# jaak-s/BayesianDataFusion.jl

Measured on AMD Instinct MI355X. Metric: Gibbs sweeps/sec (both entities) + test RMSE, MovieLens-1M D=32, higher is better.
Workload: dtype f64; 1 GPU; BPMF MovieLens-1M 6040x3952, 500209 training ratings (500000 held out), D=32, alpha=1.5, step = rows of both entities + hyperpriors + test prediction update (one native call); BEFORE the --warmup steps the engine's set-up runs 60 ms of full iterations whose results are discarded (device_warmup_ms); num_latent=32, burnin=5, psamples=1985, parallelism=1 GPU

## Files before the change

### bayesiandatafusion.jl_amd/csrc/dpp_rows32.h

```cpp
#pragma once
#include "dpp_rows16.h"

namespace {

template <int S, int I>
__device__ __forceinline__ int sys_off(int j)
{
    constexpr int IB = I / 16, ii = I % 16;
    if constexpr (IB >= S) {
        constexpr int blk = IB * (IB + 1) / 2 + S;
        return (blk * 4 + (ii >> 2)) * 64 + 16 * (ii & 3) + j;
    } else {
        return (1 * 4 + (j >> 2)) * 64 + 16 * (j & 3) + ii;
    }
}

template <int DR, int I>
__device__ __forceinline__ void col_rank1(double (&A0)[33], double (&A1)[33], double v0, double v1)
{
    if constexpr (I < 16) {
        if constexpr (I == 0) fm1<0>(A0[0], v0, v0); else fm1_run<I>(A0[I], v0, v0);
        if constexpr (16 + I < DR) {
            fm1_run<I>(A0[16 + I], v1, v0);
            fm1_run<I>(A1[16 + I], v1, v1);
        }
        col_rank1<DR, I + 1>(A0, A1, v0, v1);
    }
}
template <int DR, int S, int K, int I, bool FIRST>
__device__ __forceinline__ void fin_elim(double (&A0)[33], double (&A1)[33], double nm0, double nm1)
{
    if constexpr (I <= 32) {
        if constexpr (S == 0) {
            if constexpr (DR > 16) {
                if constexpr (FIRST) fm1<K>(A1[I], A0[I], nm1); else fm1_run<K>(A1[I], A0[I], nm1);
                fm1_self_run<K>(A0[I], nm0);
            } else {
                if constexpr (FIRST) fm1_self<K>(A0[I], nm0); else fm1_self_run<K>(A0[I], nm0);
            }
        } else {
            if constexpr (FIRST) fm1_self<K>(A1[I], nm1); else fm1_self_run<K>(A1[I], nm1);
        }
        fin_elim<DR, S, K, (I + 1 < DR || I == 32) ? I + 1 : 32, false>(A0, A1, nm0, nm1);
    }
}

template <int DR, int k>
__device__ __forceinline__ void fin_factor(double (&A0)[33], double (&A1)[33], double &d0, double &d1, int j)
{
    if constexpr (k < DR) {
        constexpr int S = k / 16, K = k % 16;
        const double dk = row_bcast_f64<K>(S ? A1[k] : A0[k]);
        const double rinv = fast_rcp(dk);
        double nm0 = 0.0, nm1;
        if constexpr (S == 0) {
            d0 = (j == K) ? dk : d0;
            nm0 = (j > K) ? -(A0[k] * rinv) : 0.0;
            nm1 = -(A1[k] * rinv);
        } else {
            d1 = (j == K) ? dk : d1;
            nm1 = (j > K) ? -(A1[k] * rinv) : 0.0;
        }
        fin_elim<DR, S, K, (k + 1 < DR) ? k + 1 : 32, true>(A0, A1, nm0, nm1);
        fin_factor<DR, k + 1>(A0, A1, d0, d1, j);
    }
}

template <int C>
__device__ __forceinline__ void fin_backward(const double (&A0)[33], const double (&A1)[33], double &y0, double &y1, double rd0,
                                             double rd1, int j)
{
    if constexpr (C >= 1) {
        constexpr int S = C / 16, K = C % 16;
        if constexpr (S == 1) {
            fm1<K>(y0, y1, -(A0[C] * rd0));
            if constexpr (K > 0) fm1_self_run<K>(y1, (j < K) ? -(A1[C] * rd1) : 0.0);
        } else {
            fm1_self<K>(y0, (j < K) ? -(A0[C] * rd0) : 0.0);
        }
        fin_backward<C - 1>(A0, A1, y0, y1, rd0, rd1, j);
    }
}

}
```

### bayesiandatafusion.jl_amd/csrc/k_rows_col.hip

```cpp
#include "rows.h"
#include "dpp_rows32.h"
#include <algorithm>

#ifndef BDF_COL_WAVES
#define BDF_COL_WAVES 2
#endif
#define COL_VGPR_HALF 104
#define COL_PSZ 800

#ifdef BDF_K1_STAMPS
#define CSTAMP_DECL unsigned long long st_t = __builtin_amdgcn_s_memtime(), st_acc = 0, st_mid = 0, st_prior = 0, st_fin = 0, st_rng = 0, st_steps = 0, st_rounds = 0, st_parts = 0, st_fins = 0, st_folds = 0; const unsigned long long st_begin = st_t
#define CSTAMP(x) do { const unsigned long long now_ = __builtin_amdgcn_s_memtime(); x += now_ - st_t; st_t = now_; } while (0)
#else
#define CSTAMP_DECL do { } while (0)
#define CSTAMP(x) do { } while (0)
#endif

namespace {

struct ColCoef { static __device__ __forceinline__ double c(double x) { asm volatile("" : "+s"(x)); return x; } };

template <int DR, int K>
__device__ __forceinline__ void col_obs(double (&A0)[33], double (&A1)[33], double v0, double v1, double r)
{
    col_rank1<DR, 0>(A0, A1, v0, v1);
    fm1_run<K>(A0[32], r, v0);
    fm1_run<K>(A1[32], r, v1);
}

__device__ __forceinline__ double col_ld(__amdgpu_buffer_rsrc_t rs, uint32_t off)
{
    typedef unsigned u2v __attribute__((ext_vector_type(2)));
    const u2v x = __builtin_amdgcn_raw_buffer_load_b64(rs, (int)off, 0, 0);
    return __hiloint2double((int)x.y, (int)x.x);
}

template <bool FULL, int K0>
__device__ __forceinline__ void col_gather4(double (&b)[4][2], __amdgpu_buffer_rsrc_t rs, uint32_t idw, uint32_t rowb, uint32_t eo, bool ok1)
{
#pragma unroll
    for (int q = 0; q < 4; q++) {
        uint32_t id;
        if (q == 0) id = row_bcast_u32<K0>(idw); else if (q == 1) id = row_bcast_u32<K0 + 1>(idw);
        else if (q == 2) id = row_bcast_u32<K0 + 2>(idw); else id = row_bcast_u32<K0 + 3>(idw);
        if constexpr (FULL) {
            const uint32_t base = id + eo;
            b[q][1] = col_ld(rs, base);
            b[q][0] = col_ld(rs, base + 128u);
        } else {
            const uint32_t base = id + eo;
            b[q][0] = col_ld(rs, base);
            b[q][1] = col_ld(rs, ok1 ? base - 128u : 0xffffffffu);
        }
    }
}
template <int DR, int K0>
__device__ __forceinline__ void col_compute4(double (&A0)[33], double (&A1)[33], const double (&b)[4][2], double r)
{
    col_obs<DR, K0>(A0, A1, b[0][0], b[0][1], r);
    col_obs<DR, K0 + 1>(A0, A1, b[1][0], b[1][1], r);
    col_obs<DR, K0 + 2>(A0, A1, b[2][0], b[2][1], r);
    col_obs<DR, K0 + 3>(A0, A1, b[3][0], b[3][1], r);
}

template <int X>
__device__ __forceinline__ void col_fold(double (&A0)[33], double (&A1)[33], double m)
{
#pragma unroll
    for (int i = 0; i < 33; i++) A0[i] = fma(__shfl_xor(A0[i], X), m, A0[i]);
#pragma unroll
    for (int i = 16; i < 33; i++) A1[i] = fma(__shfl_xor(A1[i], X), m, A1[i]);
}

template <int E0, int E1, bool ADD>
__device__ __forceinline__ void col_slot_load(double (&A0)[33], double (&A1)[33], const double *src, double m)
{
#pragma unroll
    for (int e = E0; e < E1; e++) {
        const double v = src[e * 16];
        double &d = e < 33 ? A0[e] : A1[e - 17];
        if (ADD) d = fma(v, m, d); else d = v * m;
    }
}

__device__ __forceinline__ void col_prior_dma(const double *image, unsigned lds_dst, int lane)
{
    const void *sbase = (const void *)(((uint64_t)(uint32_t)__builtin_amdgcn_readfirstlane((int)((uint64_t)image >> 32)) << 32) |
                                       (uint32_t)__builtin_amdgcn_readfirstlane((int)(uint32_t)(uint64_t)image));
#pragma unroll
    for (int k = 0; k < 6; k++) {
        const unsigned voff = (unsigned)k * 1024u + (unsigned)lane * 16u;
        unsigned keep;
        asm volatile("s_mov_b32 %0, m0\n\ts_mov_b32 m0, %2\n\ts_nop 0\n\tglobal_load_lds_dwordx4 %1, %3 sc1\n\ts_mov_b32 m0, %0"
                     : "=&s"(keep) : "v"(voff), "s"(lds_dst + (unsigned)k * 1024u), "s"(sbase) : "memory");
    }
}
template <int S, int I, int DR>
__device__ __forceinline__ void col_prior_lds(double (&A)[33], const double *img, double alpha, int j)
{
    if constexpr (I < DR) {
        A[I] = fma(alpha, A[I], img[sys_off<S, I>(j)]);
        col_prior_lds<S, I + 1, DR>(A, img, alpha, j);
    }
}

template <int DR, bool FULL>
__global__ __launch_bounds__(64, BDF_COL_WAVES) __attribute__((amdgpu_num_vgpr(COL_VGPR_HALF))) void k_rows_col(SampleArgs a_in, ColPlanDev p_in, uint32_t fac_bytes)
{
    __shared__ __attribute__((aligned(16))) double lds[4 * 272 + 768];
    const int w = blockIdx.x;
    if (w >= p_in.n_waves) return;
    const int r_end = p_in.wave_round[w + 1];
    if (a_in.span && threadIdx.x == 0) atomicMin(a_in.span + 2 * (w & 63), (unsigned long long)__builtin_amdgcn_s_memrealtime());
    CSTAMP_DECL;
#pragma nounroll
    for (int rd = p_in.wave_round[w]; rd < r_end; rd++) {
    int zero = 0, lane = threadIdx.x;
    asm volatile("" : "+s"(zero), "+v"(lane));
    const SampleArgs &a = (&a_in)[zero];
    const ColPlanDev &p = (&p_in)[zero];
    const int j = lane & 15, g = lane >> 4;
    const TermDev &T = a.t[0];
    const int D = FULL ? 32 : a.D;
    const int ec0 = D - 1 - j, ec1 = D - 17 - j;
    const int n0 = ec0, n1 = ec1 >= 0 ? ec1 : 0;
    const bool ok1 = ec1 >= 0;
    const uint32_t rowb = (uint32_t)D * 8u;
    const uint32_t eo = FULL ? (uint32_t)ec1 * 8u : (uint32_t)ec0 * 8u;
    const __amdgpu_buffer_rsrc_t rs = __builtin_amdgcn_make_buffer_rsrc((void *)T.fac[0], 0, (int)fac_bytes, 0x00020000);
    const bool coded = T.packed != nullptr;
    const double mean = T.mean;
    {
        const ColJob jb = p.jobs[(int64_t)rd * 4 + g];
        const bool live = jb.row >= 0;
        const int n = live ? jb.count : 0;
        const unsigned lds_img = (unsigned)__builtin_amdgcn_readfirstlane((int)(unsigned)(size_t)(__attribute__((address_space(3))) double *)(lds + 4 * 272));
        bool have_prior = true;
        if (a.ready) have_prior = __builtin_amdgcn_readfirstlane((int)((int32_t)(__hip_atomic_load(a.ready, __ATOMIC_RELAXED, __HIP_MEMORY_SCOPE_AGENT) - a.ready_want) >= 0)) != 0;
        if (have_prior) col_prior_dma(a.prior_c, lds_img, lane);
        double A0[33], A1[33];
#pragma unroll
        for (int i = 0; i < 33; i++) { A0[i] = 0.0; A1[i] = 0.0; }
        int nmax = n;
        nmax = max(nmax, __shfl_xor(nmax, 16));
        nmax = max(nmax, __shfl_xor(nmax, 32));
        nmax = __builtin_amdgcn_readfirstlane(nmax);
        if (nmax > 0) {
            const uint32_t *packed = coded ? T.packed + jb.q_begin : nullptr;
            const int32_t *colidx = T.colidx + jb.q_begin;
            const double *vals = T.vals + jb.q_begin;
            const double *table = T.table;
#define COL_CHUNK(c0, IDW, R)                                                                     \
            {                                                                                     \
                const int o_ = (c0) + j;                                                          \
                IDW = 0xffffffu; R = 0.0;                                                         \
                if (o_ < n) {                                                                     \
                    if (coded) { const uint32_t pw_ = packed[o_]; IDW = pw_; R = table[pw_ >> 24] - mean; } \
                    else { IDW = (uint32_t)colidx[o_]; R = vals[o_] - mean; }                     \
                }                                                                                 \
                IDW = __umul24(IDW, rowb);       \
            }
            uint32_t idw_c, idw_n;
            double r_c, r_n;
            COL_CHUNK(0, idw_c, r_c)
            double ba[4][2], bb[4][2];
            col_gather4<FULL, 0>(ba, rs, idw_c, rowb, eo, ok1);
            for (int c0 = 0;; c0 += 16) {
                COL_CHUNK(c0 + 16, idw_n, r_n)
                col_gather4<FULL, 4>(bb, rs, idw_c, rowb, eo, ok1);
                __builtin_amdgcn_sched_barrier(0);
                col_compute4<DR, 0>(A0, A1, ba, r_c);
                if (c0 + 4 >= nmax) break;
                col_gather4<FULL, 8>(ba, rs, idw_c, rowb, eo, ok1);
                __builtin_amdgcn_sched_barrier(0);
                col_compute4<DR, 4>(A0, A1, bb, r_c);
                if (c0 + 8 >= nmax) break;
                col_gather4<FULL, 12>(bb, rs, idw_c, rowb, eo, ok1);
                __builtin_amdgcn_sched_barrier(0);
                col_compute4<DR, 8>(A0, A1, ba, r_c);
                if (c0 + 12 >= nmax) break;
                col_gather4<FULL, 0>(ba, rs, idw_n, rowb, eo, ok1);
                __builtin_amdgcn_sched_barrier(0);
                col_compute4<DR, 12>(A0, A1, bb, r_c);
                if (c0 + 16 >= nmax) break;
                idw_c = idw_n; r_c = r_n;
            }
#undef COL_CHUNK
        }
#ifdef BDF_K1_STAMPS
        asm volatile("s_nop 0" :: "v"(A0[0]), "v"(A0[32]), "v"(A1[31]));
        st_steps += (unsigned long long)nmax; st_rounds++;
#endif
        CSTAMP(st_acc);
        const unsigned fl = (unsigned)jb.flags;
        if (__builtin_amdgcn_readfirstlane((int)(__ballot((fl & COLF_PAIR) != 0) != 0ull))) {
#ifdef BDF_K1_STAMPS
            st_folds++;
#endif
            col_fold<16>(A0, A1, (fl & COLF_PAIR) ? 1.0 : 0.0);
            if (__builtin_amdgcn_readfirstlane((int)(__ballot((fl & COLF_QUAD) != 0) != 0ull)))
                col_fold<32>(A0, A1, (fl & COLF_QUAD) ? 1.0 : 0.0);
        }
        if (__builtin_amdgcn_readfirstlane((int)(fl & COLF_MULTI))) {
            const int srow = __builtin_amdgcn_readfirstlane(jb.srow);
            double *dst = p.partials + (int64_t)__builtin_amdgcn_readfirstlane(jb.slot) * COL_PSZ + j;
            if (g == 0) {
#pragma unroll
                for (int e = 0; e < 33; e++) __hip_atomic_store(dst + e * 16, A0[e], __ATOMIC_RELAXED, __HIP_MEMORY_SCOPE_AGENT);
#pragma unroll
                for (int e = 33; e < 50; e++) __hip_atomic_store(dst + e * 16, A1[e - 17], __ATOMIC_RELAXED, __HIP_MEMORY_SCOPE_AGENT);
            }
            const ColSplit sr = p.rows[srow];
            asm volatile("s_waitcnt vmcnt(0)" ::: "memory");
            int old = 0;
            if (lane == 0) old = __hip_atomic_fetch_add(p.arrived + srow, 1, __ATOMIC_RELAXED, __HIP_MEMORY_SCOPE_AGENT);
            old = __builtin_amdgcn_readfirstlane(old);
#ifdef BDF_K1_STAMPS
            st_parts++;
            if (old == sr.n_slots - 1) st_fins++;
#endif
            if (old != sr.n_slots - 1) { CSTAMP(st_mid); continue; }
            __builtin_amdgcn_fence(__ATOMIC_ACQUIRE, "agent");
            asm volatile("s_waitcnt vmcnt(0)" ::: "memory");
            if (lane == 0) p.arrived[srow] = 0;
            const double *src = p.partials + (int64_t)sr.slot_begin * COL_PSZ + j;
            col_slot_load<0, 50, false>(A0, A1, src + (int64_t)(g < sr.n_slots ? g : 0) * COL_PSZ, g < sr.n_slots ? 1.0 : 0.0);
            for (int s0 = 4; s0 < sr.n_slots; s0 += 4) {
                const bool on = s0 + g < sr.n_slots;
                const double *sp = src + (int64_t)(on ? s0 + g : 0) * COL_PSZ;
                const double m = on ? 1.0 : 0.0;
                col_slot_load<0, 16, true>(A0, A1, sp, m);
                asm volatile("" ::: "memory");
                col_slot_load<16, 33, true>(A0, A1, sp, m);
                asm volatile("" ::: "memory");
                col_slot_load<33, 50, true>(A0, A1, sp, m);
                asm volatile("" ::: "memory");
            }
            col_fold<16>(A0, A1, 1.0);
            col_fold<32>(A0, A1, 1.0);
        }
        CSTAMP(st_mid);
        double z0 = 0.0, z1 = 0.0;
        {
            double ze = 0.0, zo = 0.0;
            if (live && 2 * j < D) bdf_normal_pair<ColCoef>(a.seed, a.sweep, BDF_P_ROW, a.entity_tag, (uint64_t)(uint32_t)jb.orig, (uint32_t)j, ze, zo);
            const int base = lane & 48;
            const double ze0 = __shfl(ze, base + (n0 >> 1)), zo0 = __shfl(zo, base + (n0 >> 1));
            const double ze1 = __shfl(ze, base + (n1 >> 1)), zo1 = __shfl(zo, base + (n1 >> 1));
            z0 = (n0 & 1) ? zo0 : ze0;
            z1 = ok1 ? ((n1 & 1) ? zo1 : ze1) : 0.0;
        }
        asm volatile("" ::: "memory");
        CSTAMP(st_rng);
        {
            double *tl = lds + g * 272;
#pragma unroll
            for (int r = 0; r < 16; r++) tl[r * 17 + j] = A0[16 + r];
            wave_sync();
#pragma unroll
            for (int i = 0; i < 16; i++) A1[i] = tl[j * 17 + i];
            wave_sync();
        }
        CSTAMP(st_mid);
        const double alpha = term_alpha(T);
        if (!have_prior) {
            int spins = 0;
            while ((int32_t)(__hip_atomic_load(a.ready, __ATOMIC_RELAXED, __HIP_MEMORY_SCOPE_AGENT) - a.ready_want) < 0) {
                __builtin_amdgcn_s_sleep(16);
                if (++spins > (1 << 22)) { if (lane == 0) atomicOr_system(a.flag, 16); break; }
            }
            col_prior_dma(a.prior_c, lds_img, lane);
        }
        {
            const double *pb = a.prior_b + (a.mu_is_matrix && live ? (int64_t)jb.row * D : 0);
            const double b0 = __hip_atomic_load(pb + n0, __ATOMIC_RELAXED, __HIP_MEMORY_SCOPE_AGENT);
            const double b1 = __hip_atomic_load(pb + n1, __ATOMIC_RELAXED, __HIP_MEMORY_SCOPE_AGENT);
            asm volatile("s_waitcnt vmcnt(0)" ::: "memory");
            wave_sync();
            const double *img = lds + 4 * 272;
            col_prior_lds<0, 0, DR>(A0, img, alpha, j);
            col_prior_lds<1, 0, DR>(A1, img, alpha, j);
            A0[32] = fma(alpha, A0[32], b0);
            A1[32] = ok1 ? fma(alpha, A1[32], b1) : 0.0;
            wave_sync();
        }
#ifdef BDF_K1_STAMPS
        asm volatile("s_nop 0" :: "v"(A0[0]), "v"(A0[31]), "v"(A1[0]), "v"(A1[31]));
#endif
        CSTAMP(st_prior);
        double d0 = 1.0, d1 = 1.0;
        fin_factor<DR, 0>(A0, A1, d0, d1, j);
        const bool lead = live && (fl & COLF_LEADER);
        if (lead && (!(d0 > 0.0) || (ok1 && !(d1 > 0.0)))) atomicOr_system(a.flag, 1);
        const double rd0 = fast_rcp(d0), rd1 = fast_rcp(d1);
        double y0 = fma(z0, fast_rsqrt(d0), A0[32] * rd0), y1 = fma(z1, fast_rsqrt(d1), A1[32] * rd1);
        fin_backward<DR - 1>(A0, A1, y0, y1, rd0, rd1, j);
        if (lead) __hip_atomic_store(a.out + ((int64_t)jb.row * D + ec0), y0, __ATOMIC_RELAXED, __HIP_MEMORY_SCOPE_AGENT);
        if (lead && ok1) __hip_atomic_store(a.out + ((int64_t)jb.row * D + ec1), y1, __ATOMIC_RELAXED, __HIP_MEMORY_SCOPE_AGENT);
        CSTAMP(st_fin);
    }
    }
    if (a_in.done) {
        asm volatile("s_waitcnt vmcnt(0)" ::: "memory");
        if (threadIdx.x == 0) __hip_atomic_fetch_add(a_in.done + BDF_DONE_STRIDE * (w & (BDF_DONE_SHARDS - 1)), 1u, __ATOMIC_RELAXED, __HIP_MEMORY_SCOPE_AGENT);
    }
    if (a_in.span && threadIdx.x == 0) atomicMax(a_in.span + 2 * (w & 63) + 1, (unsigned long long)__builtin_amdgcn_s_memrealtime());
#ifdef BDF_K1_STAMPS
    if (threadIdx.x == 0 && a_in.b_dump && w < 65536) {
        unsigned long long *d = (unsigned long long *)a_in.b_dump + (size_t)w * 16;
        d[0] = st_begin; d[8] = st_t; d[6] = st_rounds; d[7] = st_steps;
        d[1] = st_parts; d[2] = st_fins; d[3] = st_folds;
        d[11] = st_rng; d[12] = st_acc; d[13] = st_mid; d[14] = st_prior; d[15] = st_fin;
        d[9] = __builtin_amdgcn_s_getreg((4 - 1) << 11 | 0 << 6 | 4) | ((unsigned long long)__builtin_amdgcn_s_getreg((32 - 1) << 11 | 0 << 6 | 4));
        d[10] = __builtin_amdgcn_s_getreg((4 - 1) << 11 | 0 << 6 | 20);
    }
#endif
}

#define COL_C_OBS 56.0
#define COL_C_FIN 1460.0
#define COL_C_FOLD 180.0
#define COL_C_PART 700.0

struct Round { ColJob job[4]; double cost; };

ColJob idle_job() { return ColJob{-1, 0, 0, 0, -1, 0, 0}; }

}

int bdf_col_plan_build(bdf_ctx *ctx, const std::vector<bdf_row_ref> &rows, int T, int64_t slots, bdf_col_plan &plan)
{
    std::vector<Round> rounds;
    std::vector<ColSplit> splits;
    struct Unit { int32_t row, orig; int64_t qb; int32_t n; };
    std::vector<Unit> singles, pairs;
    int32_t n_slots_total = 0;
    auto quad_round = [&](const bdf_row_ref &rr, int64_t b0, int64_t b1, int32_t srow, int32_t slot, double fin_share) {
        Round R;
        const int64_t m = b1 - b0;
        int32_t lmax = 0;
        for (int q = 0; q < 4; q++) {
            const int64_t p0 = b0 + m * q / 4, p1 = b0 + m * (q + 1) / 4;
            R.job[q] = ColJob{rr.out, rr.orig, rr.qb + p0, (int32_t)(p1 - p0), srow, slot,
                              (int32_t)(COLF_PAIR | COLF_QUAD | (q == 0 ? COLF_LEADER : 0) | (srow >= 0 ? COLF_MULTI : 0))};
            lmax = std::max(lmax, (int32_t)(p1 - p0));
        }
        constexpr double part_extra = 3000.0;
        R.cost = COL_C_OBS * lmax + 2 * COL_C_FOLD + (srow >= 0 ? COL_C_PART + fin_share + part_extra : COL_C_FIN);
        rounds.push_back(R);
    };
    for (const bdf_row_ref &rr : rows) {
        const int64_t n = rr.cnt;
        if (n <= T) singles.push_back(Unit{rr.out, rr.orig, rr.qb, (int32_t)n});
        else if (n <= 2 * (int64_t)T) pairs.push_back(Unit{rr.out, rr.orig, rr.qb, (int32_t)n});
        else if (n <= 4 * (int64_t)T) quad_round(rr, 0, n, -1, 0, 0.0);
        else {
            const int64_t W = (n + 4 * (int64_t)T - 1) / (4 * (int64_t)T);
            BDF_REQUIRE(W < (1 << 20), BDF_ERR_ARG, "bdf_sample_rows: a row of %lld observations", (long long)n);
            const int32_t srow = (int32_t)splits.size();
            splits.push_back(ColSplit{n_slots_total, (int32_t)W});
            const double share = (COL_C_FIN + 2 * COL_C_FOLD + 60.0 * (double)((W + 3) / 4)) / (double)W;
            for (int64_t q = 0; q < W; q++) quad_round(rr, n * q / W, n * (q + 1) / W, srow, n_slots_total + (int32_t)q, share);
            n_slots_total += (int32_t)W;
        }
    }
    auto by_len = [](const Unit &x, const Unit &y) { return x.n > y.n; };
    std::stable_sort(pairs.begin(), pairs.end(), by_len);
    std::stable_sort(singles.begin(), singles.end(), by_len);
    auto pair_jobs = [](const Unit &u, ColJob *dst) {
        const int32_t h = u.n / 2;
        dst[0] = ColJob{u.row, u.orig, u.qb, h, -1, 0, COLF_PAIR | COLF_LEADER};
        dst[1] = ColJob{u.row, u.orig, u.qb + h, u.n - h, -1, 0, COLF_PAIR};
    };
    size_t si = 0;
    for (size_t pi = 0; pi < pairs.size(); pi += 2) {
        Round R;
        pair_jobs(pairs[pi], R.job);
        int32_t lmax = pairs[pi].n - pairs[pi].n / 2;
        if (pi + 1 < pairs.size()) pair_jobs(pairs[pi + 1], R.job + 2);
        else {
            for (int q = 2; q < 4; q++) {
                if (si < singles.size()) {
                    const Unit &u = singles[si++];
                    R.job[q] = ColJob{u.row, u.orig, u.qb, u.n, -1, 0, COLF_LEADER};
                    lmax = std::max(lmax, u.n);
                } else R.job[q] = idle_job();
            }
        }
        R.cost = COL_C_OBS * lmax + COL_C_FOLD + COL_C_FIN;
        rounds.push_back(R);
    }
    for (; si < singles.size(); si += 4) {
        Round R;
        for (int q = 0; q < 4; q++) {
            if (si + q < singles.size()) {
                const Unit &u = singles[si + q];
                R.job[q] = ColJob{u.row, u.orig, u.qb, u.n, -1, 0, COLF_LEADER};
            } else R.job[q] = idle_job();
        }
        R.cost = COL_C_OBS * singles[si].n + COL_C_FIN;
        rounds.push_back(R);
    }
    plan.n_rounds = (int64_t)rounds.size();
    plan.n_waves = 0;
    plan.n_split_rows = (int32_t)splits.size();
    if (rounds.empty()) return BDF_OK;
    (void)slots;
    const int64_t nw = (int64_t)rounds.size();
    std::vector<int32_t> rank(rounds.size());
    for (size_t i = 0; i < rank.size(); i++) rank[i] = (int32_t)i;
    std::stable_sort(rank.begin(), rank.end(), [&](int32_t x, int32_t y) { return rounds[(size_t)x].cost > rounds[(size_t)y].cost; });
    constexpr int64_t S2 = 896;
    std::vector<int32_t> idx;
    idx.reserve(rounds.size());
    if (nw <= S2) idx = rank;
    else {
        const int64_t two = std::min<int64_t>(nw, 2 * S2);
        const int64_t P = two - S2, A = S2 - P;
        for (int64_t i = 0; i < P; i++) idx.push_back(rank[(size_t)(A + i)]);
        for (int64_t i = 0; i < A; i++) idx.push_back(rank[(size_t)i]);
        for (int64_t i = 0; i < P; i++) idx.push_back(rank[(size_t)(two - 1 - i)]);
        for (int64_t i = two; i < nw; i++) idx.push_back(rank[(size_t)i]);
    }
    std::vector<ColJob> jobs;
    std::vector<int32_t> wave_round;
    jobs.reserve(rounds.size() * 4);
    wave_round.push_back(0);
    for (int32_t i : idx) {
        for (int q = 0; q < 4; q++) jobs.push_back(rounds[(size_t)i].job[q]);
        wave_round.push_back((int32_t)(jobs.size() / 4));
    }
    plan.cost_max = rounds[(size_t)rank.front()].cost;
    plan.cost_min = rounds[(size_t)rank.back()].cost;
    plan.n_waves = (int32_t)nw;
    BDF_HIP(hipMalloc((void **)&plan.jobs_dev, jobs.size() * sizeof(ColJob)));
    BDF_HIP(hipMemcpy(plan.jobs_dev, jobs.data(), jobs.size() * sizeof(ColJob), hipMemcpyHostToDevice));
    BDF_HIP(hipMalloc((void **)&plan.wave_round_dev, wave_round.size() * sizeof(int32_t)));
    BDF_HIP(hipMemcpy(plan.wave_round_dev, wave_round.data(), wave_round.size() * sizeof(int32_t), hipMemcpyHostToDevice));
    BDF_HIP(hipMalloc((void **)&plan.rows_dev, std::max<size_t>(splits.size() * sizeof(ColSplit), 8)));
    if (!splits.empty()) BDF_HIP(hipMemcpy(plan.rows_dev, splits.data(), splits.size() * sizeof(ColSplit), hipMemcpyHostToDevice));
    BDF_HIP(hipMalloc((void **)&plan.partials_dev, std::max<size_t>((size_t)n_slots_total * COL_PSZ * sizeof(double), 8)));
    BDF_HIP(hipMalloc((void **)&plan.arrived_dev, std::max<size_t>(splits.size() * sizeof(int32_t), 8)));
    BDF_HIP(hipMemsetAsync(plan.arrived_dev, 0, std::max<size_t>(splits.size() * sizeof(int32_t), 8), ctx->stream));
    return BDF_OK;
}

void bdf_col_plan_free(bdf_col_plan &plan)
{
    if (plan.jobs_dev) (void)hipFree(plan.jobs_dev);
    if (plan.wave_round_dev) (void)hipFree(plan.wave_round_dev);
    if (plan.rows_dev) (void)hipFree(plan.rows_dev);
    if (plan.partials_dev) (void)hipFree(plan.partials_dev);
    if (plan.arrived_dev) (void)hipFree(plan.arrived_dev);
    plan = bdf_col_plan{};
}

int bdf_col_launch(bdf_ctx *ctx, const SampleArgs &a, const bdf_col_plan &plan, int64_t M_other, hipEvent_t e0, hipEvent_t e1)
{
    if (plan.n_waves <= 0) return BDF_OK;
    ColPlanDev p;
    p.jobs = plan.jobs_dev; p.wave_round = plan.wave_round_dev; p.n_waves = plan.n_waves; p._pad = 0;
    p.rows = plan.rows_dev; p.partials = plan.partials_dev; p.arrived = plan.arrived_dev;
    const int64_t bytes = M_other * (int64_t)a.D * 8;
    BDF_REQUIRE(bytes < ((int64_t)1 << 32), BDF_ERR_ARG, "bdf_sample_rows: the column kernel needs a factor matrix below 4 GiB");
    const uint32_t fb = (uint32_t)bytes;
    const dim3 grid((unsigned)plan.n_waves), block(64);
    const int DR = (a.D + 3) / 4 * 4;
#define COL_LAUNCH(DRV, FULLV) hipExtLaunchKernelGGL((k_rows_col<DRV, FULLV>), grid, block, 0, ctx->stream, e0, e1, 0, a, p, fb)
    if (a.D == 32) COL_LAUNCH(32, true);
    else if (DR <= 20) COL_LAUNCH(20, false);
    else if (DR <= 24) COL_LAUNCH(24, false);
    else if (DR <= 28) COL_LAUNCH(28, false);
    else COL_LAUNCH(32, false);
#undef COL_LAUNCH
    BDF_HIP(hipGetLastError());
    return BDF_OK;
}
```

Measured before the change: 12950 sweeps/s.

## Pack symmetric Gram accumulator into fewer registers with star-shaped rank-1 layout

Replaces the per-lane triangular 33+17 accumulator layout with a packed 42-entry layout. Off-diagonal blocks are split across half-rows via a DPP cndmask selection, which cuts the FMAs per observation and the number of shuffle folds, partial stores and slot loads. An LDS transpose sequence after accumulation rebuilds the layout the factorization expects. This adds extra LDS traffic and wave syncs per row, and the planner's per-observation cost constant is lowered to match.

```diff
diff --git a/bayesiandatafusion.jl_amd/csrc/dpp_rows32.h b/bayesiandatafusion.jl_amd/csrc/dpp_rows32.h
--- a/bayesiandatafusion.jl_amd/csrc/dpp_rows32.h
+++ b/bayesiandatafusion.jl_amd/csrc/dpp_rows32.h
@@ -25,6 +25,37 @@
             fm1_run<I>(A1[16 + I], v1, v1);
         }
         col_rank1<DR, I + 1>(A0, A1, v0, v1);
+    }
+}
+template <int B0, int K0, int N, int I = 0>
+__device__ __forceinline__ void col_star(double (&A)[33], double s, double m)
+{
+    if constexpr (I < N) {
+        fm1_run<K0 + I>(A[B0 + I], s, m);
+        col_star<B0, K0, N, I + 1>(A, s, m);
+    }
+}
+__device__ __forceinline__ double col_own_y(double v0, double v1, uint64_t hmask)
+{
+    int lo, hi;
+    asm("s_mov_b64 vcc, %6\n\t"
+        "v_cndmask_b32_dpp %0, %2, %4, vcc row_ror:8 row_mask:0xf bank_mask:0xf\n\t"
+        "v_cndmask_b32_dpp %1, %3, %5, vcc row_ror:8 row_mask:0xf bank_mask:0xf"
+        : "=&v"(lo), "=v"(hi) : "v"(__double2loint(v0)), "v"(__double2hiint(v0)), "v"(__double2loint(v1)), "v"(__double2hiint(v1)), "s"(hmask) : "vcc");
+    return __hiloint2double(hi, lo);
+}
+template <int DR>
+__device__ __forceinline__ void col_rank1u(double (&A0)[33], double (&A1)[33], double v0, double v1, bool h, uint64_t hmask)
+{
+    fm1<0>(A0[0], v0, v0);
+    col_star<1, 1, 7>(A0, v0, v0);
+    col_star<0, 0, 8>(A1, v0, v1);
+    col_star<16, 0, (DR - 16 < 8 ? DR - 16 : 8)>(A1, v1, v1);
+    const double x = h ? v0 : v1;
+    col_star<8, 8, 8>(A0, v0, x);
+    if constexpr (DR > 24) {
+        const double y = col_own_y(v0, v1, hmask);
+        col_star<24, 8, DR - 24>(A1, v1, y);
     }
 }
 template <int DR, int S, int K, int I, bool FIRST>
diff --git a/bayesiandatafusion.jl_amd/csrc/k_rows_col.hip b/bayesiandatafusion.jl_amd/csrc/k_rows_col.hip
--- a/bayesiandatafusion.jl_amd/csrc/k_rows_col.hip
+++ b/bayesiandatafusion.jl_amd/csrc/k_rows_col.hip
@@ -6,10 +6,12 @@
 #define BDF_COL_WAVES 2
 #endif
 #define COL_VGPR_HALF 104
-#define COL_PSZ 800
-
-#ifdef BDF_K1_STAMPS
-#define CSTAMP_DECL unsigned long long st_t = __builtin_amdgcn_s_memtime(), st_acc = 0, st_mid = 0, st_prior = 0, st_fin = 0, st_rng = 0, st_steps = 0, st_rounds = 0, st_parts = 0, st_fins = 0, st_folds = 0; const unsigned long long st_begin = st_t
+#define COL_PSZ 672
+#define COL_NE 42
+#define COL_TL 304
+
+#ifdef BDF_K1_STAMPS
+#define CSTAMP_DECL unsigned long long st_t = __builtin_amdgcn_s_memtime(), st_acc = 0, st_mid = 0, st_prior = 0, st_fin = 0, st_rng = 0, st_lay = 0, st_steps = 0, st_rounds = 0, st_parts = 0, st_fins = 0, st_folds = 0; const unsigned long long st_begin = st_t
 #define CSTAMP(x) do { const unsigned long long now_ = __builtin_amdgcn_s_memtime(); x += now_ - st_t; st_t = now_; } while (0)
 #else
 #define CSTAMP_DECL do { } while (0)
@@ -21,9 +23,9 @@
 struct ColCoef { static __device__ __forceinline__ double c(double x) { asm volatile("" : "+s"(x)); return x; } };
 
 template <int DR, int K>
-__device__ __forceinline__ void col_obs(double (&A0)[33], double (&A1)[33], double v0, double v1, double r)
-{
-    col_rank1<DR, 0>(A0, A1, v0, v1);
+__device__ __forceinline__ void col_obs(double (&A0)[33], double (&A1)[33], double v0, double v1, double r, bool h, uint64_t hmask)
+{
+    col_rank1u<DR>(A0, A1, v0, v1, h, hmask);
     fm1_run<K>(A0[32], r, v0);
     fm1_run<K>(A1[32], r, v1);
 }
@@ -55,21 +57,23 @@
     }
 }
 template <int DR, int K0>
-__device__ __forceinline__ void col_compute4(double (&A0)[33], double (&A1)[33], const double (&b)[4][2], double r)
-{
-    col_obs<DR, K0>(A0, A1, b[0][0], b[0][1], r);
-    col_obs<DR, K0 + 1>(A0, A1, b[1][0], b[1][1], r);
-    col_obs<DR, K0 + 2>(A0, A1, b[2][0], b[2][1], r);
-    col_obs<DR, K0 + 3>(A0, A1, b[3][0], b[3][1], r);
-}
-
+__device__ __forceinline__ void col_compute4(double (&A0)[33], double (&A1)[33], const double (&b)[4][2], double r, bool h, uint64_t hmask)
+{
+    col_obs<DR, K0>(A0, A1, b[0][0], b[0][1], r, h, hmask);
+    col_obs<DR, K0 + 1>(A0, A1, b[1][0], b[1][1], r, h, hmask);
+    col_obs<DR, K0 + 2>(A0, A1, b[2][0], b[2][1], r, h, hmask);
+    col_obs<DR, K0 + 3>(A0, A1, b[3][0], b[3][1], r, h, hmask);
+}
+
+__device__ __forceinline__ double &col_entry(double (&A0)[33], double (&A1)[33], int e)
+{
+    return e < 16 ? A0[e] : e == 16 ? A0[32] : e < 25 ? A1[e - 17] : A1[e - 9];
+}
 template <int X>
 __device__ __forceinline__ void col_fold(double (&A0)[33], double (&A1)[33], double m)
 {
 #pragma unroll
-    for (int i = 0; i < 33; i++) A0[i] = fma(__shfl_xor(A0[i], X), m, A0[i]);
-#pragma unroll
-    for (int i = 16; i < 33; i++) A1[i] = fma(__shfl_xor(A1[i], X), m, A1[i]);
+    for (int e = 0; e < COL_NE; e++) { double &d = col_entry(A0, A1, e); d = fma(__shfl_xor(d, X), m, d); }
 }
 
 template <int E0, int E1, bool ADD>
@@ -78,7 +82,7 @@
 #pragma unroll
     for (int e = E0; e < E1; e++) {
         const double v = src[e * 16];
-        double &d = e < 33 ? A0[e] : A1[e - 17];
+        double &d = col_entry(A0, A1, e);
         if (ADD) d = fma(v, m, d); else d = v * m;
     }
 }
@@ -107,7 +111,7 @@
 template <int DR, bool FULL>
 __global__ __launch_bounds__(64, BDF_COL_WAVES) __attribute__((amdgpu_num_vgpr(COL_VGPR_HALF))) void k_rows_col(SampleArgs a_in, ColPlanDev p_in, uint32_t fac_bytes)
 {
-    __shared__ __attribute__((aligned(16))) double lds[4 * 272 + 768];
+    __shared__ __attribute__((aligned(16))) double lds[4 * COL_TL + 768];
     const int w = blockIdx.x;
     if (w >= p_in.n_waves) return;
     const int r_end = p_in.wave_round[w + 1];
@@ -120,6 +124,8 @@
     const SampleArgs &a = (&a_in)[zero];
     const ColPlanDev &p = (&p_in)[zero];
     const int j = lane & 15, g = lane >> 4;
+    const bool hh = (j & 8) != 0;
+    const uint64_t hmask = 0xff00ff00ff00ff00ull;
     const TermDev &T = a.t[0];
     const int D = FULL ? 32 : a.D;
     const int ec0 = D - 1 - j, ec1 = D - 17 - j;
@@ -134,7 +140,7 @@
         const ColJob jb = p.jobs[(int64_t)rd * 4 + g];
         const bool live = jb.row >= 0;
         const int n = live ? jb.count : 0;
-        const unsigned lds_img = (unsigned)__builtin_amdgcn_readfirstlane((int)(unsigned)(size_t)(__attribute__((address_space(3))) double *)(lds + 4 * 272));
+        const unsigned lds_img = (unsigned)__builtin_amdgcn_readfirstlane((int)(unsigned)(size_t)(__attribute__((address_space(3))) double *)(lds + 4 * COL_TL));
         bool have_prior = true;
         if (a.ready) have_prior = __builtin_amdgcn_readfirstlane((int)((int32_t)(__hip_atomic_load(a.ready, __ATOMIC_RELAXED, __HIP_MEMORY_SCOPE_AGENT) - a.ready_want) >= 0)) != 0;
         if (have_prior) col_prior_dma(a.prior_c, lds_img, lane);
@@ -169,19 +175,19 @@
                 COL_CHUNK(c0 + 16, idw_n, r_n)
                 col_gather4<FULL, 4>(bb, rs, idw_c, rowb, eo, ok1);
                 __builtin_amdgcn_sched_barrier(0);
-                col_compute4<DR, 0>(A0, A1, ba, r_c);
+                col_compute4<DR, 0>(A0, A1, ba, r_c, hh, hmask);
                 if (c0 + 4 >= nmax) break;
                 col_gather4<FULL, 8>(ba, rs, idw_c, rowb, eo, ok1);
                 __builtin_amdgcn_sched_barrier(0);
-                col_compute4<DR, 4>(A0, A1, bb, r_c);
+                col_compute4<DR, 4>(A0, A1, bb, r_c, hh, hmask);
                 if (c0 + 8 >= nmax) break;
                 col_gather4<FULL, 12>(bb, rs, idw_c, rowb, eo, ok1);
                 __builtin_amdgcn_sched_barrier(0);
-                col_compute4<DR, 8>(A0, A1, ba, r_c);
+                col_compute4<DR, 8>(A0, A1, ba, r_c, hh, hmask);
                 if (c0 + 12 >= nmax) break;
                 col_gather4<FULL, 0>(ba, rs, idw_n, rowb, eo, ok1);
                 __builtin_amdgcn_sched_barrier(0);
-                col_compute4<DR, 12>(A0, A1, bb, r_c);
+                col_compute4<DR, 12>(A0, A1, bb, r_c, hh, hmask);
                 if (c0 + 16 >= nmax) break;
                 idw_c = idw_n; r_c = r_n;
             }
@@ -206,9 +212,7 @@
             double *dst = p.partials + (int64_t)__builtin_amdgcn_readfirstlane(jb.slot) * COL_PSZ + j;
             if (g == 0) {
 #pragma unroll
-                for (int e = 0; e < 33; e++) __hip_atomic_store(dst + e * 16, A0[e], __ATOMIC_RELAXED, __HIP_MEMORY_SCOPE_AGENT);
-#pragma unroll
-                for (int e = 33; e < 50; e++) __hip_atomic_store(dst + e * 16, A1[e - 17], __ATOMIC_RELAXED, __HIP_MEMORY_SCOPE_AGENT);
+                for (int e = 0; e < COL_NE; e++) __hip_atomic_store(dst + e * 16, col_entry(A0, A1, e), __ATOMIC_RELAXED, __HIP_MEMORY_SCOPE_AGENT);
             }
             const ColSplit sr = p.rows[srow];
             asm volatile("s_waitcnt vmcnt(0)" ::: "memory");
@@ -224,16 +228,16 @@
             asm volatile("s_waitcnt vmcnt(0)" ::: "memory");
             if (lane == 0) p.arrived[srow] = 0;
             const double *src = p.partials + (int64_t)sr.slot_begin * COL_PSZ + j;
-            col_slot_load<0, 50, false>(A0, A1, src + (int64_t)(g < sr.n_slots ? g : 0) * COL_PSZ, g < sr.n_slots ? 1.0 : 0.0);
+            col_slot_load<0, COL_NE, false>(A0, A1, src + (int64_t)(g < sr.n_slots ? g : 0) * COL_PSZ, g < sr.n_slots ? 1.0 : 0.0);
             for (int s0 = 4; s0 < sr.n_slots; s0 += 4) {
                 const bool on = s0 + g < sr.n_slots;
                 const double *sp = src + (int64_t)(on ? s0 + g : 0) * COL_PSZ;
                 const double m = on ? 1.0 : 0.0;
-                col_slot_load<0, 16, true>(A0, A1, sp, m);
+                col_slot_load<0, 14, true>(A0, A1, sp, m);
                 asm volatile("" ::: "memory");
-                col_slot_load<16, 33, true>(A0, A1, sp, m);
+                col_slot_load<14, 28, true>(A0, A1, sp, m);
                 asm volatile("" ::: "memory");
-                col_slot_load<33, 50, true>(A0, A1, sp, m);
+                col_slot_load<28, COL_NE, true>(A0, A1, sp, m);
                 asm volatile("" ::: "memory");
             }
             col_fold<16>(A0, A1, 1.0);
@@ -250,18 +254,54 @@
             z0 = (n0 & 1) ? zo0 : ze0;
             z1 = ok1 ? ((n1 & 1) ? zo1 : ze1) : 0.0;
         }
-        asm volatile("" ::: "memory");
+        asm volatile("" : "+v"(z0), "+v"(z1) :: "memory");
         CSTAMP(st_rng);
         {
-            double *tl = lds + g * 272;
-#pragma unroll
-            for (int r = 0; r < 16; r++) tl[r * 17 + j] = A0[16 + r];
+            double *tl = lds + g * COL_TL;
+            const int jl = j & 7;
+            if (!hh) {
+#pragma unroll
+                for (int i = 0; i < 8; i++) tl[jl * 9 + i] = A0[8 + i];
+#pragma unroll
+                for (int i = 0; i < 8; i++) tl[72 + i * 9 + jl] = A1[24 + i];
+            }
+            {
+                double *w = tl + 144 + (hh ? 72 : 0) + jl * 9;
+#pragma unroll
+                for (int i = 0; i < 8; i++) w[i] = A1[i];
+            }
             wave_sync();
-#pragma unroll
-            for (int i = 0; i < 16; i++) A1[i] = tl[j * 17 + i];
+            {
+                const double *r2 = tl + (hh ? 72 : 0) + jl * 9;
+                const double *r3 = tl + (hh ? 0 : 144) + jl;
+                const double *r4 = tl + (hh ? 72 : 216) + jl;
+#pragma unroll
+                for (int i = 0; i < 8; i++) A1[8 + i] = r2[i];
+#pragma unroll
+                for (int i = 0; i < 8; i++) if (16 + i < DR) A0[16 + i] = r3[i * 9];
+#pragma unroll
+                for (int i = 0; i < 8; i++) if (24 + i < DR) A0[24 + i] = r4[i * 9];
+            }
             wave_sync();
-        }
-        CSTAMP(st_mid);
+            if (hh) {
+#pragma unroll
+                for (int i = 0; i < 8; i++) tl[jl * 9 + i] = A0[i];
+#pragma unroll
+                for (int i = 0; i < 8; i++) tl[72 + jl * 9 + i] = A1[16 + i];
+            }
+            wave_sync();
+            if (!hh) {
+#pragma unroll
+                for (int i = 0; i < 8; i++) A0[8 + i] = tl[i * 9 + jl];
+#pragma unroll
+                for (int i = 0; i < 8; i++) if (24 + i < DR) A1[24 + i] = tl[72 + i * 9 + jl];
+            }
+            wave_sync();
+        }
+#ifdef BDF_K1_STAMPS
+        asm volatile("s_waitcnt lgkmcnt(0)\n\ts_nop 0" :: "v"(A0[8]), "v"(A0[31]), "v"(A1[8]), "v"(A1[31]));
+#endif
+        CSTAMP(st_lay);
         const double alpha = term_alpha(T);
         if (!have_prior) {
             int spins = 0;
@@ -277,7 +317,7 @@
             const double b1 = __hip_atomic_load(pb + n1, __ATOMIC_RELAXED, __HIP_MEMORY_SCOPE_AGENT);
             asm volatile("s_waitcnt vmcnt(0)" ::: "memory");
             wave_sync();
-            const double *img = lds + 4 * 272;
+            const double *img = lds + 4 * COL_TL;
             col_prior_lds<0, 0, DR>(A0, img, alpha, j);
             col_prior_lds<1, 0, DR>(A1, img, alpha, j);
             A0[32] = fma(alpha, A0[32], b0);
@@ -309,7 +349,7 @@
     if (threadIdx.x == 0 && a_in.b_dump && w < 65536) {
         unsigned long long *d = (unsigned long long *)a_in.b_dump + (size_t)w * 16;
         d[0] = st_begin; d[8] = st_t; d[6] = st_rounds; d[7] = st_steps;
-        d[1] = st_parts; d[2] = st_fins; d[3] = st_folds;
+        d[1] = st_parts; d[2] = st_fins; d[3] = st_folds; d[4] = st_lay;
         d[11] = st_rng; d[12] = st_acc; d[13] = st_mid; d[14] = st_prior; d[15] = st_fin;
         d[9] = __builtin_amdgcn_s_getreg((4 - 1) << 11 | 0 << 6 | 4) | ((unsigned long long)__builtin_amdgcn_s_getreg((32 - 1) << 11 | 0 << 6 | 4));
         d[10] = __builtin_amdgcn_s_getreg((4 - 1) << 11 | 0 << 6 | 20);
@@ -317,7 +357,7 @@
 #endif
 }
 
-#define COL_C_OBS 56.0
+#define COL_C_OBS 52.0
 #define COL_C_FIN 1460.0
 #define COL_C_FOLD 180.0
 #define COL_C_PART 700.0
```

Result: faster. 13560 sweeps/s, median of 6 (+4.7%).
